# radoslawkrolikowski/financial-market-data-analysis

Hardware: NVIDIA B200
Metric: sequences/sec (train step) biGRU h=256 seq=128 feat=64 (higher is better)
Workload: dtype bf16x3 (fp32-class: split bf16 operand pairs on tensor cores, fp32 accumulate / state / gradients)

## Files before the change

financial_market_data_analysis_b200/csrc/path_x3.cuh:

```cuda
#pragma once
#include "path_bf16.cuh"
#include "tc_scan_x.cuh"
#include <cstdlib>

static int x3_plan_check(const bigru_plan& p) {
    if ((p.H != 128 && p.H != 256) || p.B % 32 != 0) {
        bigru_set_error("BIGRU_PREC_BF16X3 supports hidden_size 128 or 256 and batch %% 32 == 0 (got H=%d B=%d; the Python mirror pads "
                        "other batch sizes with zero rows); use BIGRU_PREC_FP32 for other shapes", p.H, p.B);
        return BIGRU_ERR_UNSUPPORTED;
    }
    return BIGRU_OK;
}

struct X3Layout {
    size_t Yhi[16], Ylo[16], YB[16], G[16], Xhi[16], Xlo[16];
    size_t Wih_hi[16], Wih_lo[16], WihT_hi[16], WihT_lo[16], Wimg[16], WTimg[16], bfold[16], bhn[16];
    size_t cat, arg, dbg, stash_total;
    size_t gi, dghn_hi, dghn_lo, dYa, dYb, gh0, scratch_total;
};
static X3Layout x3_layout(const bigru_plan& p) {
    X3Layout L{};
    const size_t R = (size_t)p.B * p.T, DH = (size_t)p.D * p.H, H = p.H, D = p.D;
    size_t o = 0;
    for (int l = 0; l < p.L; ++l) {
        const size_t I = p.in_size(l), Ip = (size_t)pad8((int64_t)I);
        L.Yhi[l] = o; o = al(o + R * DH * 2);
        L.Ylo[l] = o; o = al(o + R * DH * 2);
        L.YB[l] = o; o = al(o + R * DH * 4);
        L.G[l] = o; o = al(o + R * D * 4 * H * 4);
        L.Xhi[l] = o; o = al(o + R * Ip * 2);
        L.Xlo[l] = o; o = al(o + R * Ip * 2);
        L.Wih_hi[l] = o; o = al(o + D * 3 * H * Ip * 2);
        L.Wih_lo[l] = o; o = al(o + D * 3 * H * Ip * 2);
        L.WihT_hi[l] = o; o = al(o + D * 3 * H * I * 2);
        L.WihT_lo[l] = o; o = al(o + D * 3 * H * I * 2);
        L.Wimg[l] = o; o = al(o + D * 2 * 3 * H * H * 2);
        L.WTimg[l] = o; o = al(o + D * 2 * 3 * H * H * 2);
        L.bfold[l] = o; o = al(o + D * 3 * H * 4);
        L.bhn[l] = o; o = al(o + D * H * 4);
    }
    L.cat = o; o = al(o + (size_t)p.B * 3 * H * 4);
    L.arg = o; o = al(o + (size_t)p.B * H * 4);
    L.dbg = o; o = al(o + 256);
    L.stash_total = o;
    o = 0;
    const size_t wide = DH > (size_t)p.F ? DH : (size_t)p.F;
    L.gi = o; o = al(o + R * D * 3 * H * 4);
    L.dghn_hi = o; o = al(o + R * D * H * 2);
    L.dghn_lo = o; o = al(o + R * D * H * 2);
    L.dYa = o; o = al(o + R * wide * 4);
    L.dYb = o; o = al(o + R * wide * 4);
    L.gh0 = o; o = al(o + (size_t)p.B * D * 3 * H * 4);
    L.scratch_total = o;
    return L;
}
static void x3_workspace(const bigru_plan& p, size_t* a, size_t* b) {
    const X3Layout L = x3_layout(p);
    *a = L.stash_total; *b = L.scratch_total;
}

__device__ __forceinline__ void x3_split(float x, bf16_t& hi, bf16_t& lo) {
    hi = __float2bfloat16(x);
    lo = __float2bfloat16(x - __bfloat162float(hi));
}

__global__ void x3_dropout_rows_kernel(const bf16_t* __restrict__ Yhi, const bf16_t* __restrict__ Ylo, bf16_t* __restrict__ Xhi,
                                       bf16_t* __restrict__ Xlo, int64_t R, int cols, int B, int T, float pdrop, uint64_t seed, uint32_t stream) {
    const float scale = 1.f / (1.f - pdrop);
    const int64_t total = R * cols;
    for (int64_t i = (int64_t)blockIdx.x * blockDim.x + threadIdx.x; i < total; i += (int64_t)gridDim.x * blockDim.x) {
        const int cidx = i % cols;
        const int64_t r = i / cols;
        const int64_t b = r % B, t = r / B;
        const uint64_t key = ((uint64_t)b * T + t) * cols + cidx;
        const float v = bigru_uniform(seed, stream, key) < pdrop ? 0.f : (__bfloat162float(Yhi[i]) + __bfloat162float(Ylo[i])) * scale;
        bf16_t hi, lo;
        x3_split(v, hi, lo);
        Xhi[i] = hi; Xlo[i] = lo;
    }
}
__global__ void x3_dropout_grad_rows_kernel(float* __restrict__ dYB, int64_t R, int cols, int B, int T, int H, float pdrop,
                                            uint64_t seed, uint32_t stream) {
    const float scale = 1.f / (1.f - pdrop);
    const int64_t total = R * cols;
    const int CS = H / 64, ntl = B / 32;
    for (int64_t i = (int64_t)blockIdx.x * blockDim.x + threadIdx.x; i < total; i += (int64_t)gridDim.x * blockDim.x) {
        const int i8 = i & 7;
        int64_t e = i >> 3;
        const int tid = e % 256; e /= 256;
        const int c = e % CS; e /= CS;
        const int t = e % T; e /= T;
        const int tile = e % ntl;
        const int d = e / ntl;
        const int unit = c * 64 + (tid & 63);
        const int64_t b = tile * 32 + (tid >> 6) * 8 + i8;
        const uint64_t key = ((uint64_t)b * T + t) * cols + (uint64_t)(d * H + unit);
        dYB[i] = bigru_uniform(seed, stream, key) < pdrop ? 0.f : dYB[i] * scale;
    }
}

struct X3PackJob { const float* w_ih; const float* w_hh; const float* b_ih; const float* b_hh;
                   bf16_t *Wih_hi, *Wih_lo, *WihT_hi, *WihT_lo, *Wimg, *WTimg; float* bfold; float* bhn; int I; int d; };
struct X3PackJobs { X3PackJob j[32]; };
__global__ void __launch_bounds__(256) x3_pack_all_kernel(const X3PackJobs jobs, int H, int D) {
    __shared__ float tile[32][33];
    const X3PackJob& J = jobs.j[blockIdx.y];
    const int H3 = 3 * H, I = J.I, d = J.d;
    const int tx = threadIdx.x & 31, ty = threadIdx.x >> 5;
    if (I % 32 == 0) {
        const int tr = H3 / 32, tcn = I / 32;
        for (int tl = blockIdx.x; tl < tr * tcn; tl += gridDim.x) {
            const int r0 = (tl / tcn) * 32, c0 = (tl % tcn) * 32;
#pragma unroll
            for (int i = ty; i < 32; i += 8) {
                const float v = J.w_ih[(int64_t)(r0 + i) * I + c0 + tx];
                tile[i][tx] = v;
                bf16_t hi, lo;
                x3_split(v, hi, lo);
                const int64_t o = ((int64_t)d * H3 + r0 + i) * I + c0 + tx;
                J.Wih_hi[o] = hi; J.Wih_lo[o] = lo;
            }
            __syncthreads();
#pragma unroll
            for (int i = ty; i < 32; i += 8) {
                bf16_t hi, lo;
                x3_split(tile[tx][i], hi, lo);
                const int64_t o = (int64_t)(c0 + i) * D * H3 + (int64_t)d * H3 + r0 + tx;
                J.WihT_hi[o] = hi; J.WihT_lo[o] = lo;
            }
            __syncthreads();
        }
    } else {
        const int Ip = (I + 7) & ~7;
        const int64_t n_ih = (int64_t)H3 * Ip;
        for (int64_t i = (int64_t)blockIdx.x * blockDim.x + threadIdx.x; i < n_ih; i += (int64_t)gridDim.x * blockDim.x) {
            const int k = i % Ip, q = i / Ip;
            bf16_t hi, lo;
            x3_split(k < I ? J.w_ih[(int64_t)q * I + k] : 0.f, hi, lo);
            const int64_t o1 = ((int64_t)d * H3 + q) * Ip + k, o2 = (int64_t)k * D * H3 + (int64_t)d * H3 + q;
            J.Wih_hi[o1] = hi; J.Wih_lo[o1] = lo;
            if (k < I) { J.WihT_hi[o2] = hi; J.WihT_lo[o2] = lo; }
        }
    }
    {
        const int CS = H / 64, NKH = H / 128, NRB = 2 * NKH;
        const int64_t per_cta = (int64_t)128 * 3 * H;
        const int64_t total = (int64_t)CS * per_cta;
        bf16_t* fimg = J.Wimg + (int64_t)d * total;
        bf16_t* bimg = J.WTimg + (int64_t)d * total;
        for (int64_t i = (int64_t)blockIdx.x * blockDim.x + threadIdx.x; i < total; i += (int64_t)gridDim.x * blockDim.x) {
            const int c = (int)(i / per_cta);
            const int64_t r = i % per_cta;
            {
                const int row = (int)(r / (3 * H)), col = (int)(r % (3 * H));
                const int g = col / H, k = col % H, part = row >> 6, jj = row & 63;
                bf16_t hi, lo;
                x3_split(J.w_hh[((int64_t)g * H + 64 * c + jj) * H + k], hi, lo);
                fimg[i] = part ? lo : hi;
            }
            {
                const int lane_i = (int)(r / (NRB * 192)), col = (int)(r % (NRB * 192));
                const int rb = col / 192, kq = col % 192, g = kq / 64, jj = kq % 64;
                const int part = rb / NKH, kh = rb % NKH;
                bf16_t hi, lo;
                x3_split(J.w_hh[((int64_t)g * H + 64 * c + jj) * H + 128 * kh + lane_i], hi, lo);
                bimg[i] = part ? lo : hi;
            }
        }
    }
    for (int64_t q = (int64_t)blockIdx.x * blockDim.x + threadIdx.x; q < H3; q += (int64_t)gridDim.x * blockDim.x) {
        J.bfold[d * H3 + q] = J.b_ih[q] + (q < 2 * H ? J.b_hh[q] : 0.f);
        if (q >= 2 * H) J.bhn[d * H + q - 2 * H] = J.b_hh[q];
    }
}

static int forward_x3(const bigru_plan& p, const float* params, const float* x, const float* h0, float drop,
                      int spatial, int training, uint64_t seed, void* stash_v, void* scratch_v, float* logits,
                      float* hn, cudaStream_t st, WindowSrc win = WindowSrc{nullptr, nullptr, nullptr, 0}) {
    const X3Layout L = x3_layout(p);
    uint8_t* S = (uint8_t*)stash_v;
    uint8_t* W = (uint8_t*)scratch_v;
    const int B = p.B, T = p.T, H = p.H, D = p.D, F = p.F;
    const int64_t R = (int64_t)B * T;
    const bool do_drop = training && drop > 0.f;
    unsigned int* dbg = (unsigned int*)(S + L.dbg);
    CUDA_TRY(cudaMemsetAsync(dbg, 0, 64, st));
    {
        X3PackJobs jobs{};
        int nj = 0;
        for (int l = 0; l < p.L; ++l)
            for (int d = 0; d < D; ++d) {
                X3PackJob& J = jobs.j[nj++];
                J.w_ih = params + p.off_wih(l, d); J.w_hh = params + p.off_whh(l, d);
                J.b_ih = params + p.off_bih(l, d); J.b_hh = params + p.off_bhh(l, d);
                J.Wih_hi = (bf16_t*)(S + L.Wih_hi[l]); J.Wih_lo = (bf16_t*)(S + L.Wih_lo[l]);
                J.WihT_hi = (bf16_t*)(S + L.WihT_hi[l]); J.WihT_lo = (bf16_t*)(S + L.WihT_lo[l]);
                J.Wimg = (bf16_t*)(S + L.Wimg[l]); J.WTimg = (bf16_t*)(S + L.WTimg[l]);
                J.bfold = (float*)(S + L.bfold[l]); J.bhn = (float*)(S + L.bhn[l]); J.I = (int)p.in_size(l); J.d = d;
            }
        KLAUNCH(KC_PACK, 0.0, 0.0, st, x3_pack_all_kernel<<<dim3(148, nj), 256, 0, st>>>(jobs, H, D));
    }
    const bool direct = windows_direct(p, win.src != nullptr, do_drop);
    if (direct)
        KLAUNCH(KC_PACK, 0.0, 8.0 * (B + T - 1) * F, st, chunk_prep_kernel<<<148, 256, 0, st>>>(win, (bf16_t*)(S + L.Xhi[0]), (bf16_t*)(S + L.Xlo[0]),
                                                                                                 (int64_t)B + T - 1, F));
    else if (F % 8 == 0)
        KLAUNCH(KC_PACK, 0.0, 8.0 * R * F, st, cast_x_kernel<<<148 * 8, 256, 0, st>>>(x, win, (bf16_t*)(S + L.Xhi[0]), (bf16_t*)(S + L.Xlo[0]), B, T, F,
                                                                                       do_drop ? drop : 0.f, spatial, seed));
    else
        KLAUNCH(KC_PACK, 0.0, 8.0 * R * F, st, cast_x_pad_kernel<<<148 * 8, 256, 0, st>>>(x, win, (bf16_t*)(S + L.Xhi[0]), (bf16_t*)(S + L.Xlo[0]), B, T, F,
                                                                                           pad8(F), do_drop ? drop : 0.f, spatial, seed));
    for (int l = 0; l < p.L; ++l) {
        const int I = (int)p.in_size(l);
        const bf16_t* Xhi = (const bf16_t*)(S + L.Xhi[l]);
        const bf16_t* Xlo = (const bf16_t*)(S + L.Xlo[l]);
        if (l > 0) {
            if (do_drop) {
                KLAUNCH(KC_MISC, 0.0, 0.0, st, x3_dropout_rows_kernel<<<148 * 8, 256, 0, st>>>(
                                                   (const bf16_t*)(S + L.Yhi[l - 1]), (const bf16_t*)(S + L.Ylo[l - 1]), (bf16_t*)(S + L.Xhi[l]),
                                                   (bf16_t*)(S + L.Xlo[l]), R, I, B, T, drop, seed, (uint32_t)l));
            } else {
                Xhi = (const bf16_t*)(S + L.Yhi[l - 1]); Xlo = (const bf16_t*)(S + L.Ylo[l - 1]);
            }
        }
        {
            tcg::Params g{};
            const int Ip = pad8(I);
            g.M = D * 3 * H; g.N = (int)R; g.K = Ip; g.batch = 1; g.splitk = 1; g.mode = tcg::OUT_SCAN_F32;
            g.blk = tcg::ScanBlk{T, B, H, 3, 64, 32}; g.m_fast = 1;
            g.C = W + L.gi; g.ldc = R; g.bias = (const float*)(S + L.bfold[l]); g.bias_per_row = 1; g.dbg = dbg;
            const bool wnd = direct && l == 0;
            g.b_win = wnd ? B : 0;
            TRY(tc_gemm(S + L.Wih_hi[l], D * 3 * H, Ip, Xhi, wnd ? (int64_t)B + T - 1 : R, Ip, g, st, KC_TC_GEMM, S + L.Wih_lo[l], Xlo));
        }
        if (h0) {
            GemmArgs r = gemm_args(h0 + (int64_t)l * D * B * H, params + p.off_whh(l, 0), (float*)(W + L.gh0), B, 3 * H, H, H, 1, H, 1, 3 * H);
            r.batch = D; r.zA = (int64_t)B * H; r.zB = p.ld_block(l); r.zC = (int64_t)B * 3 * H;
            TRY(sgemm_launch(r, st));
        }
        tcx::FwdParams f{};
        f.B = B; f.T = T; f.H = H; f.D = D;
        f.Wimg = (const bf16_t*)(S + L.Wimg[l]); f.giX = (const float*)(W + L.gi); f.b_hn = (const float*)(S + L.bhn[l]);
        f.h0 = h0 ? h0 + (int64_t)l * D * B * H : nullptr;
        f.gh0 = h0 ? (const float*)(W + L.gh0) : nullptr;
        f.GX = (float*)(S + L.G[l]); f.YBX = (float*)(S + L.YB[l]);
        f.hn_out = hn ? hn + (int64_t)l * D * B * H : nullptr;
        f.Yhi = (bf16_t*)(S + L.Yhi[l]); f.Ylo = (bf16_t*)(S + L.Ylo[l]); f.dbg = dbg;
        {
            ProfScope ps(KC_TC_SCAN_FWD, 2.0 * 3 * H * H * (double)R * D, 0.0, st);
            CUDA_TRY(tcx::launch_fwd(f, st));
        }
    }
    {
        const int G = 256 / (H / 8);
        const size_t hsm = sizeof(float) * ((size_t)3 * G * H + (size_t)p.C * 8);
        KLAUNCH(KC_HEAD, 0.0, 4.0 * R * D * H, st, head_fwd_kernel<<<B, 256, hsm, st>>>(
                    (const bf16_t*)(S + L.Yhi[p.L - 1]), (const bf16_t*)(S + L.Ylo[p.L - 1]), params + p.off_linw(), params + p.off_linb(),
                    (float*)(S + L.cat), (int*)(S + L.arg), logits, B, T, H, D, p.C));
    }
    return BIGRU_OK;
}

static int backward_x3(const bigru_plan& p, const float* params, const float* x, const float* h0, float drop,
                       int spatial, int training, uint64_t seed, const void* stash_v, void* scratch_v,
                       const float* dlogits, float* grads, float* dx, float* dh0, cudaStream_t st, int l_from = -1, int l_to = 0) {
    if (l_from < 0) l_from = p.L - 1;
    const bool from_top = l_from == p.L - 1;
    const X3Layout L = x3_layout(p);
    const uint8_t* S = (const uint8_t*)stash_v;
    uint8_t* W = (uint8_t*)scratch_v;
    const int B = p.B, T = p.T, H = p.H, D = p.D, C = p.C;
    const int64_t R = (int64_t)B * T;
    const bool do_drop = training && drop > 0.f;
    unsigned int* dbg = (unsigned int*)(const_cast<uint8_t*>(S) + L.dbg);
    if (from_top) CUDA_TRY(cudaMemsetAsync(grads, 0, sizeof(float) * p.nparams, st));
    const float* cat = (const float*)(S + L.cat);
    if (from_top) {
        const int bchunk = 16;
        KLAUNCH(KC_HEAD, 0.0, 0.0, st, head_bwd_w_kernel<<<dim3(nblk2(3 * H, 128), C, (B + bchunk - 1) / bchunk), 128, 0, st>>>(
                    dlogits, cat, grads + p.off_linw(), grads + p.off_linb(), B, 3 * H, C, bchunk));
    }
    float* dY = (float*)(W + L.dYa);
    float* dYnext = (float*)(W + L.dYb);
    if ((p.L - 1 - l_from) & 1) { float* t_ = dY; dY = dYnext; dYnext = t_; }
    bf16_t* dgi_hi = (bf16_t*)(W + L.gi);
    bf16_t* dgi_lo = dgi_hi + (size_t)R * D * 3 * H;
    bf16_t* dghn_hi = (bf16_t*)(W + L.dghn_hi);
    bf16_t* dghn_lo = (bf16_t*)(W + L.dghn_lo);
    for (int l = l_from; l >= l_to; --l) {
        const int I = (int)p.in_size(l);
        tcx::BwdParams b{};
        b.B = B; b.T = T; b.H = H; b.D = D;
        b.WTimg = (const bf16_t*)(S + L.WTimg[l]); b.GX = (const float*)(S + L.G[l]); b.YBX = (const float*)(S + L.YB[l]);
        b.dYBX = dY;
        b.h0 = h0 ? h0 + (int64_t)l * D * B * H : nullptr;
        b.dh0 = dh0 ? dh0 + (int64_t)l * D * B * H : nullptr;
        if (l == p.L - 1) { b.dlogits = dlogits; b.lin_w = params + p.off_linw(); b.arg = (const int*)(S + L.arg); b.C = C; }
        b.dgi_hi = dgi_hi; b.dgi_lo = dgi_lo; b.dghn_hi = dghn_hi; b.dghn_lo = dghn_lo;
        b.db_ih = grads + p.off_bih(l, 0); b.db_hh = grads + p.off_bhh(l, 0); b.dir_stride = p.ld_block(l); b.dbg = dbg;
        {
            ProfScope ps(KC_TC_SCAN_BWD, 2.0 * 3 * H * H * (double)R * D, 0.0, st);
            CUDA_TRY(tcx::launch_bwd(b, st));
        }
        const bool dropped = do_drop && (l == 0 || p.L > 1);
        const bool own_x = l == 0 || dropped;
        const bf16_t* Xin_hi = own_x ? (const bf16_t*)(S + L.Xhi[l]) : (const bf16_t*)(S + L.Yhi[l - 1]);
        const bf16_t* Xin_lo = own_x ? (const bf16_t*)(S + L.Xlo[l]) : (const bf16_t*)(S + L.Ylo[l - 1]);
        {
            tcg::Params g{};
            g.M = 3 * H; g.N = I; g.K = (int)R; g.batch = D; g.mode = tcg::OUT_ATOMIC_F32; g.a_mn = 1; g.b_mn = 1;
            const int tiles = ((3 * H + 127) / 128) * ((I + 127) / 128) * D;
            g.splitk = (int)std::max<int64_t>(1, std::min<int64_t>((R + 63) / 64, (148 * 2 + tiles / 2) / tiles));
            g.C = grads + p.off_wih(l, 0); g.ldc = I; g.zC = p.ld_block(l);
            for (int d = 0; d < D; ++d) { g.a_row_off[d] = d * 3 * H; g.b_row_off[d] = 0; g.b_k_off[d] = 0; }
            g.dbg = dbg;
            g.b_win = (l == 0 && windows_direct(p, x == nullptr, do_drop)) ? B : 0;
            g.b_win_rows = B + T - 1;
            TRY(tc_gemm(dgi_hi, (int64_t)D * 3 * H, (int64_t)D * 3 * H, Xin_hi, I, pad8(I), g, st, KC_TC_GEMM_DWIH, dgi_lo, Xin_lo));
        }
        for (int part = 0; part < 2; ++part) {
            tcg::Params g{};
            g.M = part == 0 ? 2 * H : H; g.N = H; g.K = (int)R; g.batch = D; g.mode = tcg::OUT_ATOMIC_F32; g.a_mn = 1; g.b_mn = 1;
            const int tiles = ((g.M + 127) / 128) * ((H + 127) / 128) * D;
            g.splitk = (int)std::max<int64_t>(1, std::min<int64_t>((R + 63) / 64, (148 * 2 + tiles / 2) / tiles));
            g.C = grads + p.off_whh(l, 0) + (part == 0 ? 0 : (int64_t)2 * H * H); g.ldc = H; g.zC = p.ld_block(l);
            for (int d = 0; d < D; ++d) {
                g.a_row_off[d] = part == 0 ? d * 3 * H : d * H;
                g.b_row_off[d] = d * H; g.b_k_off[d] = d == 0 ? -B : B;
            }
            g.dbg = dbg;
            if (part == 0) TRY(tc_gemm(dgi_hi, (int64_t)D * 3 * H, (int64_t)D * 3 * H, S + L.Yhi[l], (int64_t)D * H, (int64_t)D * H, g, st, KC_TC_GEMM_DWHH, dgi_lo, S + L.Ylo[l]));
            else TRY(tc_gemm(dghn_hi, (int64_t)D * H, (int64_t)D * H, S + L.Yhi[l], (int64_t)D * H, (int64_t)D * H, g, st, KC_TC_GEMM_DWHH, dghn_lo, S + L.Ylo[l]));
        }
        if (h0)
            KLAUNCH(KC_MISC, 0.0, 0.0, st, dwhh_h0_kernel<<<dim3((3 * H + 127) / 128, H / DWHH_H0_COLS, D), 128, 0, st>>>(
                        dgi_hi, dgi_lo, dghn_hi, dghn_lo, h0 + (int64_t)l * D * B * H, grads + p.off_whh(l, 0), p.ld_block(l), B, T, H, D));
        const bool need_dx = l > 0 || dx != nullptr;
        if (need_dx) {
            tcg::Params g{};
            g.M = I; g.N = (int)R; g.K = D * 3 * H; g.batch = 1; g.splitk = 1;
            g.mode = l > 0 ? tcg::OUT_SCAN_F32 : tcg::OUT_F32;
            g.blk = tcg::ScanBlk{T, B, H, 1, 64, 32}; g.m_fast = 1;
            g.C = dYnext; g.ldc = R; g.dbg = dbg;
            TRY(tc_gemm(S + L.WihT_hi[l], I, (int64_t)D * 3 * H, dgi_hi, R, (int64_t)D * 3 * H, g, st, KC_TC_GEMM_DX, S + L.WihT_lo[l], dgi_lo));
            if (l > 0 && dropped)
                KLAUNCH(KC_MISC, 0.0, 0.0, st, x3_dropout_grad_rows_kernel<<<148 * 8, 256, 0, st>>>(dYnext, R, I, B, T, H, drop, seed, (uint32_t)l));
            if (l == 0) {
                dim3 grid((I + 31) / 32, (B + 31) / 32, T);
                KLAUNCH(KC_MISC, 0.0, 0.0, st, dx_to_batch_major_kernel<<<grid, dim3(32, 8), 0, st>>>(dYnext, dx, B, T, I,
                                                                                               do_drop ? drop : 0.f, spatial, seed));
            }
        }
        float* tmp = dY; dY = dYnext; dYnext = tmp;
    }
    return BIGRU_OK;
}
```

financial_market_data_analysis_b200/csrc/tc_gemm.cuh:

```cuda
#pragma once
#include "tc_common.cuh"
#include <cstring>

namespace tcg {

constexpr int BM = 128, BN = 128, BK = 64, MAX_STAGES = 4;
constexpr int A_BYTES = BM * BK * 2, B_BYTES = BN * BK * 2;
static inline int smem_bytes_for(int stages, int stage_out = 65536) {
    const int ring = stages * (A_BYTES + B_BYTES);
    return (ring < stage_out ? stage_out : ring) + 1024  + 256 ;
}
constexpr int THREADS = 192;

enum { OUT_F32 = 0, OUT_BF16 = 1, OUT_ATOMIC_F32 = 2, OUT_SCAN_BF16 = 3, OUT_SCAN_F32 = 4 };

struct ScanBlk { int T, B, H, G; int U, NB; };

struct Params {
    int M, N, K;
    int batch, splitk;
    int mode;
    void* C; int64_t ldc;
    int64_t zC;
    int a_row_off[4], b_row_off[4], b_k_off[4];
// ... 84 lines not shown
                if (++s == STAGES) { s = 0; ph ^= 1; }
            }
        }
    } else if (warp == 1) {
        if (tc::elect_one()) {
            const uint32_t idesc = tc::umma_idesc_bf16(BM, BN, (uint32_t)p.a_mn, (uint32_t)p.b_mn);
            const int nit = nkb * p.nsplit;
            int s = 0;
            uint32_t ph = 0;
            for (int i = 0; i < nit; ++i, s = (s + 1 == STAGES ? 0 : s + 1), ph ^= (s == 0 ? 1u : 0u)) {
                if (!tc::mbar_wait(&full[s], ph, p.dbg, 0x200 + s)) break;
                tc::tcgen05_fence_after();
                const uint32_t aa = tc::smem_u32(sA + s * A_BYTES), ab = tc::smem_u32(sB + s * B_BYTES);
                const uint64_t da = p.a_mn ? tc::umma_desc_mn_sw128(aa, A_BYTES / 2) : tc::umma_desc_k_sw128(aa);
                const uint64_t db = p.b_mn ? tc::umma_desc_mn_sw128(ab, B_BYTES / 2) : tc::umma_desc_k_sw128(ab);
                const uint64_t sa = p.a_mn ? 128 : 2, sb = p.b_mn ? 128 : 2;
#pragma unroll
                for (int kk = 0; kk < BK / 16; ++kk)
                    tc::umma_bf16(tmem, da + sa * kk, db + sb * kk, idesc, (i | kk) ? 1u : 0u);
                tc::umma_commit(&empty[s]);
            }
            tc::umma_commit(accum);
        }
    } else {
        const int q = warp & 3;
        const int m = m0 + q * 32 + lane;
        bool ok = tc::mbar_wait(accum, 0, p.dbg, 0x300);
        tc::tcgen05_fence_after();
        const float* bias = p.bias ? p.bias + z * p.zBias : nullptr;
        const float brow = (bias && p.bias_per_row && m < p.M) ? bias[m] : 0.f;
        if (ok && p.mode >= OUT_SCAN_BF16 && p.tma_store) {
            const int ml = q * 32 + lane;
            const bool bf = p.mode == OUT_SCAN_BF16;
            const int run_bytes = bf ? 2048 : 4096;
#pragma unroll 1
            for (int c = 0; c < BN / 32; ++c) {
                uint32_t v[32];
                if (nkb > 0) { tc::tmem_ld32(tmem + ((uint32_t)(q * 32) << 16) + c * 32, v); tc::tmem_ld_wait(); }
                else {
#pragma unroll
                    for (int i = 0; i < 32; ++i) v[i] = 0u;
                }
                const int nb = n0 + c * 32;
#pragma unroll
                for (int i8 = 0; i8 < 32; i8 += 8) {
                    float f[8];
#pragma unroll
                    for (int j = 0; j < 8; ++j)
                        f[j] = __uint_as_float(v[i8 + j]) + (bias ? (p.bias_per_row ? brow : ((nb + i8 + j < p.N) ? bias[nb + i8 + j] : 0.f)) : 0.f);
                    uint8_t* dst = smem + (size_t)(c * 4 + (i8 >> 3)) * run_bytes;
                    if (bf) {
                        uint32_t w[4];
#pragma unroll
                        for (int j = 0; j < 4; ++j) {
                            __nv_bfloat162 h2 = __floats2bfloat162_rn(f[2 * j], f[2 * j + 1]);
                            w[j] = *reinterpret_cast<uint32_t*>(&h2);
                        }
                        tc::sts_u4(tc::smem_u32(dst) + ml * 16, make_uint4(w[0], w[1], w[2], w[3]));
                    } else {
                        tc::sts_f4(tc::smem_u32(dst) + ml * 32, make_float4(f[0], f[1], f[2], f[3]));
                        tc::sts_f4(tc::smem_u32(dst) + ml * 32 + 16, make_float4(f[4], f[5], f[6], f[7]));
                    }
                }
            }
            tc::fence_proxy_async_smem();
            asm volatile("bar.sync 1, 128;" ::: "memory");
            if (warp == 2 && tc::elect_one()) {
                const int H = p.blk.H, G = p.blk.G, Bb = p.blk.B, Tt = p.blk.T, U = p.blk.U;
                const int sh = p.blk.NB == 32 ? 5 : 4;
                const int CSs = H / U, ntl = Bb >> sh, nh = BM / U;
                const size_t es = bf ? 2 : 4;
                size_t row_part[2]; size_t gate_part[2];
                for (int hh = 0; hh < nh; ++hh) {
                    const int mr = m0 + hh * U;
                    row_part[hh] = (size_t)(mr / (G * H)) * ntl;
                    gate_part[hh] = (size_t)((mr % H) / U) * G + (size_t)((mr / H) % G);
                }
                int t_ = n0 / Bb, b = n0 % Bb;
                for (int r = 0; r < BN / 8; ++r) {
                    if (n0 + r * 8 >= p.N) break;
                    const int tile_ = b >> sh, cbg = (b & ((1 << sh) - 1)) >> 3;
                    for (int hh = 0; hh < nh; ++hh) {
                        const size_t e = ((((row_part[hh] + tile_) * Tt + t_) * CSs * G + gate_part[hh]) * 256 + (size_t)cbg * U) * 8;
                        tc::bulk_s2g(reinterpret_cast<uint8_t*>(p.C) + e * es, smem + (size_t)r * run_bytes + (size_t)hh * U * 8 * es,
                                     (uint32_t)(U * 8 * es));
                    }
                    b += 8;
                    if (b >= Bb) { b -= Bb; ++t_; }
                }
                tc::tma_store_commit();
                tc::tma_store_wait_read();
            }
        } else if (ok && p.tma_store) {
            const int ml = q * 32 + lane;
            const uint32_t sw = (uint32_t)(ml & 7);
            const bool is_bf16 = p.mode == OUT_BF16;
#pragma unroll 1
            for (int c = 0; c < BN / 32; ++c) {
                uint32_t v[32];
                if (nkb > 0) {
                    tc::tmem_ld32(tmem + ((uint32_t)(q * 32) << 16) + c * 32, v);
                    tc::tmem_ld_wait();
                } else {
#pragma unroll
                    for (int i = 0; i < 32; ++i) v[i] = 0u;
                }
                const int nb = n0 + c * 32;
                if (bias && ks == 0) {
#pragma unroll
                    for (int i = 0; i < 32; ++i) {
                        const float bb = p.bias_per_row ? brow : ((nb + i < p.N) ? bias[nb + i] : 0.f);
                        v[i] = __float_as_uint(__uint_as_float(v[i]) + bb);
                    }
                }
                if (is_bf16) {
                    uint8_t* box = smem + (size_t)(c >> 1) * 16384 + (size_t)ml * 128;
#pragma unroll
                    for (int k4 = 0; k4 < 4; ++k4) {
                        uint32_t w[4];
#pragma unroll
                        for (int j = 0; j < 4; ++j) {
                            __nv_bfloat162 h2 = __floats2bfloat162_rn(__uint_as_float(v[k4 * 8 + 2 * j]), __uint_as_float(v[k4 * 8 + 2 * j + 1]));
                            w[j] = *reinterpret_cast<uint32_t*>(&h2);
                        }
                        const uint32_t chunk = ((uint32_t)((c & 1) * 4 + k4)) ^ sw;
                        tc::sts_u4(tc::smem_u32(box) + chunk * 16, make_uint4(w[0], w[1], w[2], w[3]));
                    }
                } else {
                    uint8_t* box = smem + (size_t)c * 16384 + (size_t)ml * 128;
#pragma unroll
                    for (int k4 = 0; k4 < 8; ++k4) {
                        const uint32_t chunk = ((uint32_t)k4) ^ sw;
                        tc::sts_u4(tc::smem_u32(box) + chunk * 16, make_uint4(v[k4 * 4], v[k4 * 4 + 1], v[k4 * 4 + 2], v[k4 * 4 + 3]));
                    }
                }
            }
            tc::fence_proxy_async_smem();
            asm volatile("bar.sync 1, 128;" ::: "memory");
            if (warp == 2 && tc::elect_one()) {
                const int nboxes = is_bf16 ? BN / 64 : BN / 32;
                const int bw = is_bf16 ? 64 : 32;
                for (int b = 0; b < nboxes; ++b) {
                    if (n0 + b * bw >= p.N) break;
                    if (p.mode == OUT_ATOMIC_F32) {
                        if (z == 0) tc::tma_reduce_add_2d(&tmC0, smem + (size_t)b * 16384, n0 + b * bw, m0);
                        else tc::tma_reduce_add_2d(&tmC1, smem + (size_t)b * 16384, n0 + b * bw, m0);
                    } else {
                        if (z == 0) tc::tma_store_2d(&tmC0, smem + (size_t)b * 16384, n0 + b * bw, m0);
                        else tc::tma_store_2d(&tmC1, smem + (size_t)b * 16384, n0 + b * bw, m0);
                    }
                }
                tc::tma_store_commit();
                tc::tma_store_wait_read();
            }
        } else if (ok) {
#pragma unroll 1
            for (int c = 0; c < BN / 32; ++c) {
                uint32_t v[32];
                if (nkb > 0) {
                    tc::tmem_ld32(tmem + ((uint32_t)(q * 32) << 16) + c * 32, v);
                    tc::tmem_ld_wait();
                } else {
#pragma unroll
                    for (int i = 0; i < 32; ++i) v[i] = 0u;
                }
                const int nb = n0 + c * 32;
                if (m < p.M && nb < p.N && p.mode >= OUT_SCAN_BF16) {
                    const int H = p.blk.H, G = p.blk.G, Bb = p.blk.B, Tt = p.blk.T, U = p.blk.U, NBt = p.blk.NB;
                    const int dd = m / (G * H), gg = (m / H) % G, unit = m % H;
                    const int CSs = H / U, cc = unit / U, ju = unit % U;
                    const int ntl = Bb / NBt;
#pragma unroll
                    for (int i8 = 0; i8 < 32; i8 += 8) {
                        const int n = nb + i8;
                        if (n >= p.N) break;
                        const int t = n / Bb, b = n % Bb;
                        const int tile = b / NBt;
                        const int tid = ju + U * ((b % NBt) >> 3);
                        const size_t e = ((((((size_t)dd * ntl + tile) * Tt + t) * CSs + cc) * G + gg) * 256 + tid) * 8;
                        float f[8];
#pragma unroll
                        for (int j = 0; j < 8; ++j) f[j] = __uint_as_float(v[i8 + j]) + (bias ? (p.bias_per_row ? brow : bias[n + j]) : 0.f);
                        if (p.mode == OUT_SCAN_BF16) {
                            uint32_t w[4];
#pragma unroll
                            for (int j = 0; j < 4; ++j) {
                                __nv_bfloat162 h2 = __floats2bfloat162_rn(f[2 * j], f[2 * j + 1]);
                                w[j] = *reinterpret_cast<uint32_t*>(&h2);
                            }
                            *reinterpret_cast<uint4*>(reinterpret_cast<__nv_bfloat16*>(p.C) + e) = make_uint4(w[0], w[1], w[2], w[3]);
                        } else {
                            float4* o = reinterpret_cast<float4*>(reinterpret_cast<float*>(p.C) + e);
                            o[0] = make_float4(f[0], f[1], f[2], f[3]);
                            o[1] = make_float4(f[4], f[5], f[6], f[7]);
                        }
                    }
                } else if (m < p.M && nb < p.N) {
                    if (p.mode == OUT_BF16) {
                        __nv_bfloat16* crow = reinterpret_cast<__nv_bfloat16*>(p.C) + z * p.zC + (int64_t)m * p.ldc + nb;
                        if (nb + 32 <= p.N && (p.ldc % 8 == 0)) {
#pragma unroll
                            for (int i = 0; i < 32; i += 8) {
                                uint32_t w[4];
#pragma unroll
                                for (int j = 0; j < 4; ++j) {
                                    float a = __uint_as_float(v[i + 2 * j]), b = __uint_as_float(v[i + 2 * j + 1]);
                                    if (bias) {
                                        if (p.bias_per_row) { a += brow; b += brow; }
                                        else { a += bias[nb + i + 2 * j]; b += bias[nb + i + 2 * j + 1]; }
                                    }
                                    __nv_bfloat162 h2 = __floats2bfloat162_rn(a, b);
                                    w[j] = *reinterpret_cast<uint32_t*>(&h2);
                                }
                                *reinterpret_cast<uint4*>(crow + i) = make_uint4(w[0], w[1], w[2], w[3]);
                            }
                        } else {
                            for (int i = 0; i < 32 && nb + i < p.N; ++i) {
                                float a = __uint_as_float(v[i]);
                                if (bias) a += p.bias_per_row ? brow : bias[nb + i];
                                crow[i] = __float2bfloat16(a);
                            }
                        }
                    } else {
                        float* crow = reinterpret_cast<float*>(p.C) + z * p.zC + (int64_t)m * p.ldc + nb;
                        for (int i = 0; i < 32 && nb + i < p.N; ++i) {
                            float a = __uint_as_float(v[i]);
                            if (bias && ks == 0) a += p.bias_per_row ? brow : bias[nb + i];
                            if (p.mode == OUT_ATOMIC_F32) atomicAdd(crow + i, a);
                            else crow[i] = a;
                        }
                    }
                }
            }
        }
    }
    tc::tcgen05_fence_before();
    __syncthreads();
    if (warp == 1) tc::tmem_dealloc(tmem, BN);
}

static inline int make_operand_map(CUtensorMap* m, const void* base, uint64_t rows, uint64_t K, uint64_t ld) {
    const uint64_t dims[2] = {K, rows};
    const uint64_t strides[1] = {ld * 2};
    const uint32_t box[2] = {(uint32_t)BK, 128u};
    return make_tmap_bf16(m, base, 2, dims, strides, box);
}

static inline int make_output_map(CUtensorMap* m, void* base, int mode, uint64_t M, uint64_t N, uint64_t ldc) {
    const bool bf = mode == OUT_BF16;
    const uint64_t dims[2] = {N, M};
    const uint64_t strides[1] = {ldc * (bf ? 2u : 4u)};
    const uint32_t box[2] = {bf ? 64u : 32u, 128u};
    return make_tmap_typed(m, bf ? CU_TENSOR_MAP_DATA_TYPE_BFLOAT16 : CU_TENSOR_MAP_DATA_TYPE_FLOAT32, base, 2, dims, strides, box);
}

static inline int make_operand_map_mn(CUtensorMap* m, const void* base, uint64_t Krows, uint64_t MN, uint64_t ld) {
    const uint64_t dims[2] = {MN, Krows};
    const uint64_t strides[1] = {ld * 2};
    const uint32_t box[2] = {64u, (uint32_t)BK};
    return make_tmap_bf16(m, base, 2, dims, strides, box);
}

static inline cudaError_t launch(const CUtensorMap& tmA, const CUtensorMap& tmB, const Params& p_in, cudaStream_t st,
                                 const CUtensorMap* tmAlo = nullptr, const CUtensorMap* tmBlo = nullptr) {
    {
        static bool attr_set[64] = {};
        int dev = 0;
        cudaGetDevice(&dev);
        if (dev < 0 || dev >= 64 || !attr_set[dev]) {
            cudaError_t e = cudaFuncSetAttribute(gemm_kernel, cudaFuncAttributeMaxDynamicSharedMemorySize, smem_bytes_for(MAX_STAGES));
            if (e != cudaSuccess) return e;
            if (dev >= 0 && dev < 64) attr_set[dev] = true;
        }
    }
    Params p = p_in;
    if (p.nsplit != 3 || !tmAlo || !tmBlo) p.nsplit = 1;
    if (p.blk.U == 0) { p.blk.U = 128; p.blk.NB = 16; }
    {
        const int kblocks = (((p.K + BK - 1) / BK + p.splitk - 1) / p.splitk) * p.nsplit;
        p.stages = kblocks <= 2 ? kblocks : (kblocks <= 12 ? 2 : 3);
        if (p.stages < 1) p.stages = 1;
    }
    CUtensorMap tmC[2];
    memset(tmC, 0, sizeof(tmC));
    const size_t es = p.mode == OUT_BF16 ? 2 : 4;
    const bool scan_mode = p.mode >= OUT_SCAN_BF16;
    bool tma_ok = !scan_mode && p.batch <= 2 && ((p.ldc * es) % 16 == 0) && ((p.zC * es) % 16 == 0) && ((uintptr_t)p.C % 16 == 0);
    if (tma_ok) {
        for (int z = 0; z < p.batch; ++z)
            if (make_output_map(&tmC[z], (uint8_t*)p.C + (size_t)z * p.zC * es, p.mode, (uint64_t)p.M, (uint64_t)p.N, (uint64_t)p.ldc) != 0) tma_ok = false;
        if (p.batch == 1) tmC[1] = tmC[0];
    }
    p.tma_store = tma_ok ? 1 : 0;
    if (scan_mode && p.M % BM == 0 && p.blk.H % p.blk.U == 0 && p.blk.B % p.blk.NB == 0 && ((uintptr_t)p.C % 16 == 0)) p.tma_store = 1;
    dim3 grid((p.N + BN - 1) / BN, (p.M + BM - 1) / BM, p.batch * p.splitk);
    if (p.m_fast) { const unsigned t = grid.x; grid.x = grid.y; grid.y = t; }
    const int stage_out = p.tma_store ? ((p.mode == OUT_BF16 || p.mode == OUT_SCAN_BF16) ? 32768 : 65536) : 0;
    gemm_kernel<<<grid, THREADS, smem_bytes_for(p.stages, stage_out), st>>>(tmA, tmB, p.nsplit == 3 ? *tmAlo : tmA, p.nsplit == 3 ? *tmBlo : tmB,
                                                                            tmC[0], tmC[1], p);
    return cudaGetLastError();
}

}
```

Baseline: 164,300.

## Add persistent stream-K bf16x3 GEMM kernel for backward weight and dx GEMMs

Adds a dedicated persistent bf16x3 GEMM kernel with one CTA per SM. Its scheduler uses stream-K for atomic-accumulate outputs and grid-stride over tiles otherwise, with a double-buffered TMEM accumulator so the epilogue overlaps the next tile's MMAs. The two dW_hh GEMMs (r/z gates from dgi, n gate from dghn) are merged into one launch through a second A operand selected by row offset. The dW_ih and dx GEMMs are routed through the new kernel. This is meant to cut split-K launch and wave-quantization overhead and to save a launch, at the cost of a new kernel path with fixed stage counts and 1 CTA/SM occupancy.

After: 154,100, median of 6. -6.2%, worse.

```diff
diff --git a/financial_market_data_analysis_b200/csrc/path_x3.cuh b/financial_market_data_analysis_b200/csrc/path_x3.cuh
--- a/financial_market_data_analysis_b200/csrc/path_x3.cuh
+++ b/financial_market_data_analysis_b200/csrc/path_x3.cuh
@@ -174,6 +174,28 @@
     }
 }
 
+struct X3Operand { const void* hi; const void* lo; int64_t rows, ld; };
+static int x3_operand_map(CUtensorMap* m, const void* base, int mn, int64_t rows, int64_t kext, int64_t ld) {
+    const int e = mn ? tcg::make_operand_map_mn(m, base, (uint64_t)kext, (uint64_t)rows, (uint64_t)ld)
+                     : tcg::make_operand_map(m, base, (uint64_t)rows, (uint64_t)kext, (uint64_t)ld);
+    if (e) bigru_set_error("cuTensorMapEncodeTiled failed (rows %lld K %lld ld %lld)", (long long)rows, (long long)kext, (long long)ld);
+    return e;
+}
+static int tc_gemm_x3(const X3Operand& A, const X3Operand& Bo, tcg::X3Params& p, cudaStream_t st, int kclass,
+                      const X3Operand& A2 = X3Operand{nullptr, nullptr, 0, 0}) {
+    CUtensorMap tA, tAl, tB, tBl, tA2, tA2l;
+    const int64_t bk = p.b_mn && p.b_win ? p.b_win_rows : p.K;
+    if (x3_operand_map(&tA, A.hi, p.a_mn, A.rows, p.K, A.ld) || x3_operand_map(&tAl, A.lo, p.a_mn, A.rows, p.K, A.ld) ||
+        x3_operand_map(&tB, Bo.hi, p.b_mn, Bo.rows, bk, Bo.ld) || x3_operand_map(&tBl, Bo.lo, p.b_mn, Bo.rows, bk, Bo.ld))
+        return BIGRU_ERR_CUDA;
+    const bool a2 = A2.hi != nullptr;
+    if (a2 && (x3_operand_map(&tA2, A2.hi, p.a_mn, A2.rows, p.K, A2.ld) || x3_operand_map(&tA2l, A2.lo, p.a_mn, A2.rows, p.K, A2.ld)))
+        return BIGRU_ERR_CUDA;
+    ProfScope ps(kclass, 2.0 * p.M * p.N * (double)p.K * p.batch, 0.0, st);
+    CUDA_TRY(tcg::launch_x3(tA, tAl, tB, tBl, a2 ? &tA2 : nullptr, a2 ? &tA2l : nullptr, p, st));
+    return BIGRU_OK;
+}
+
 static int forward_x3(const bigru_plan& p, const float* params, const float* x, const float* h0, float drop,
                       int spatial, int training, uint64_t seed, void* stash_v, void* scratch_v, float* logits,
                       float* hn, cudaStream_t st, WindowSrc win = WindowSrc{nullptr, nullptr, nullptr, 0}) {
@@ -307,42 +329,41 @@
         const bf16_t* Xin_hi = own_x ? (const bf16_t*)(S + L.Xhi[l]) : (const bf16_t*)(S + L.Yhi[l - 1]);
         const bf16_t* Xin_lo = own_x ? (const bf16_t*)(S + L.Xlo[l]) : (const bf16_t*)(S + L.Ylo[l - 1]);
         {
-            tcg::Params g{};
+            tcg::X3Params g{};
             g.M = 3 * H; g.N = I; g.K = (int)R; g.batch = D; g.mode = tcg::OUT_ATOMIC_F32; g.a_mn = 1; g.b_mn = 1;
-            const int tiles = ((3 * H + 127) / 128) * ((I + 127) / 128) * D;
-            g.splitk = (int)std::max<int64_t>(1, std::min<int64_t>((R + 63) / 64, (148 * 2 + tiles / 2) / tiles));
             g.C = grads + p.off_wih(l, 0); g.ldc = I; g.zC = p.ld_block(l);
             for (int d = 0; d < D; ++d) { g.a_row_off[d] = d * 3 * H; g.b_row_off[d] = 0; g.b_k_off[d] = 0; }
             g.dbg = dbg;
             g.b_win = (l == 0 && windows_direct(p, x == nullptr, do_drop)) ? B : 0;
             g.b_win_rows = B + T - 1;
-            TRY(tc_gemm(dgi_hi, (int64_t)D * 3 * H, (int64_t)D * 3 * H, Xin_hi, I, pad8(I), g, st, KC_TC_GEMM_DWIH, dgi_lo, Xin_lo));
-        }
-        for (int part = 0; part < 2; ++part) {
-            tcg::Params g{};
-            g.M = part == 0 ? 2 * H : H; g.N = H; g.K = (int)R; g.batch = D; g.mode = tcg::OUT_ATOMIC_F32; g.a_mn = 1; g.b_mn = 1;
-            const int tiles = ((g.M + 127) / 128) * ((H + 127) / 128) * D;
-            g.splitk = (int)std::max<int64_t>(1, std::min<int64_t>((R + 63) / 64, (148 * 2 + tiles / 2) / tiles));
-            g.C = grads + p.off_whh(l, 0) + (part == 0 ? 0 : (int64_t)2 * H * H); g.ldc = H; g.zC = p.ld_block(l);
+            TRY(tc_gemm_x3(X3Operand{dgi_hi, dgi_lo, (int64_t)D * 3 * H, (int64_t)D * 3 * H}, X3Operand{Xin_hi, Xin_lo, I, pad8(I)},
+                           g, st, KC_TC_GEMM_DWIH));
+        }
+        {
+            tcg::X3Params g{};
+            g.M = 3 * H; g.N = H; g.K = (int)R; g.batch = D; g.mode = tcg::OUT_ATOMIC_F32; g.a_mn = 1; g.b_mn = 1;
+            g.C = grads + p.off_whh(l, 0); g.ldc = H; g.zC = p.ld_block(l);
+            g.a2_m = 2 * H;
             for (int d = 0; d < D; ++d) {
-                g.a_row_off[d] = part == 0 ? d * 3 * H : d * H;
+                g.a_row_off[d] = d * 3 * H; g.a2_row_off[d] = d * H;
                 g.b_row_off[d] = d * H; g.b_k_off[d] = d == 0 ? -B : B;
             }
             g.dbg = dbg;
-            if (part == 0) TRY(tc_gemm(dgi_hi, (int64_t)D * 3 * H, (int64_t)D * 3 * H, S + L.Yhi[l], (int64_t)D * H, (int64_t)D * H, g, st, KC_TC_GEMM_DWHH, dgi_lo, S + L.Ylo[l]));
-            else TRY(tc_gemm(dghn_hi, (int64_t)D * H, (int64_t)D * H, S + L.Yhi[l], (int64_t)D * H, (int64_t)D * H, g, st, KC_TC_GEMM_DWHH, dghn_lo, S + L.Ylo[l]));
+            TRY(tc_gemm_x3(X3Operand{dgi_hi, dgi_lo, (int64_t)D * 3 * H, (int64_t)D * 3 * H}, X3Operand{S + L.Yhi[l], S + L.Ylo[l], (int64_t)D * H, (int64_t)D * H},
+                           g, st, KC_TC_GEMM_DWHH, X3Operand{dghn_hi, dghn_lo, (int64_t)D * H, (int64_t)D * H}));
         }
         if (h0)
             KLAUNCH(KC_MISC, 0.0, 0.0, st, dwhh_h0_kernel<<<dim3((3 * H + 127) / 128, H / DWHH_H0_COLS, D), 128, 0, st>>>(
                         dgi_hi, dgi_lo, dghn_hi, dghn_lo, h0 + (int64_t)l * D * B * H, grads + p.off_whh(l, 0), p.ld_block(l), B, T, H, D));
         const bool need_dx = l > 0 || dx != nullptr;
         if (need_dx) {
-            tcg::Params g{};
+            tcg::X3Params g{};
             g.M = I; g.N = (int)R; g.K = D * 3 * H; g.batch = 1; g.splitk = 1;
             g.mode = l > 0 ? tcg::OUT_SCAN_F32 : tcg::OUT_F32;
             g.blk = tcg::ScanBlk{T, B, H, 1, 64, 32}; g.m_fast = 1;
             g.C = dYnext; g.ldc = R; g.dbg = dbg;
-            TRY(tc_gemm(S + L.WihT_hi[l], I, (int64_t)D * 3 * H, dgi_hi, R, (int64_t)D * 3 * H, g, st, KC_TC_GEMM_DX, S + L.WihT_lo[l], dgi_lo));
+            TRY(tc_gemm_x3(X3Operand{S + L.WihT_hi[l], S + L.WihT_lo[l], I, (int64_t)D * 3 * H}, X3Operand{dgi_hi, dgi_lo, R, (int64_t)D * 3 * H},
+                           g, st, KC_TC_GEMM_DX));
             if (l > 0 && dropped)
                 KLAUNCH(KC_MISC, 0.0, 0.0, st, x3_dropout_grad_rows_kernel<<<148 * 8, 256, 0, st>>>(dYnext, R, I, B, T, H, drop, seed, (uint32_t)l));
             if (l == 0) {
diff --git a/financial_market_data_analysis_b200/csrc/tc_gemm.cuh b/financial_market_data_analysis_b200/csrc/tc_gemm.cuh
--- a/financial_market_data_analysis_b200/csrc/tc_gemm.cuh
+++ b/financial_market_data_analysis_b200/csrc/tc_gemm.cuh
@@ -410,3 +410,5 @@
 }
 
 }
+
+#include "tc_gemm_x3.cuh"
diff --git a/financial_market_data_analysis_b200/csrc/tc_gemm_x3.cuh b/financial_market_data_analysis_b200/csrc/tc_gemm_x3.cuh
--- /dev/null
+++ b/financial_market_data_analysis_b200/csrc/tc_gemm_x3.cuh
@@ -0,0 +1,295 @@
+#pragma once
+#include "tc_gemm.cuh"
+
+namespace tcg {
+
+struct X3Params : Params {
+    int a2_m;
+    int a2_row_off[4];
+};
+
+constexpr int X3_TILE = BM * BK * 2;
+constexpr int X3_STAGE_BYTES = 4 * X3_TILE;
+constexpr int X3_STG_BYTES = 16384;
+constexpr int X3_DATA = 3 * X3_STAGE_BYTES + 2 * X3_STG_BYTES;
+constexpr int X3_SMEM = X3_DATA + 1024  + 256 ;
+static_assert(X3_SMEM <= 227 * 1024 && X3_DATA == 2 * X3_STAGE_BYTES + 6 * X3_STG_BYTES, "x3 GEMM shared memory");
+constexpr int X3_SHORT_KB = 8;
+constexpr int X3_SK_PIECE = 128;
+
+struct X3Sched {
+    int tiles_m, tiles_n, kbt, slices;
+    int64_t ntile;
+    int64_t pos, end, stride;
+    bool sk;
+    __device__ __forceinline__ X3Sched(const X3Params& p) {
+        tiles_m = (p.M + BM - 1) / BM; tiles_n = (p.N + BN - 1) / BN; kbt = (p.K + BK - 1) / BK;
+        ntile = (int64_t)tiles_m * tiles_n * p.batch;
+        sk = p.mode == OUT_ATOMIC_F32;
+        slices = 1;
+        if (sk) {
+            slices = (int)min((int64_t)kbt, (gridDim.x + ntile - 1) / ntile);
+            const int64_t total = ntile * kbt;
+            pos = total * blockIdx.x / gridDim.x; end = total * (blockIdx.x + 1) / gridDim.x; stride = 0;
+        } else {
+            pos = blockIdx.x; end = ntile; stride = gridDim.x;
+        }
+    }
+    __device__ __forceinline__ bool next(const X3Params& p, int& z, int& m0, int& n0, int& kb0, int& nkb) {
+        int64_t tile;
+        if (sk) {
+            if (pos >= end) return false;
+            const int64_t q = pos / ntile;
+            const int sl = (int)min((int64_t)slices - 1, ((q + 1) * slices - 1) / kbt);
+            const int ks0 = (int)((int64_t)sl * kbt / slices), ks1 = (int)((int64_t)(sl + 1) * kbt / slices);
+            const int64_t r = pos - ntile * ks0;
+            tile = r / (ks1 - ks0);
+            const int kl = (int)(r % (ks1 - ks0));
+            kb0 = ks0 + kl;
+            nkb = (int)min((int64_t)min(ks1 - ks0 - kl, X3_SK_PIECE), end - pos);
+            pos += nkb;
+        } else {
+            if (pos >= end) return false;
+            tile = pos; kb0 = 0; nkb = kbt;
+            pos += stride;
+        }
+        int mt, nt;
+        if (p.m_fast) { mt = (int)(tile % tiles_m); tile /= tiles_m; nt = (int)(tile % tiles_n); tile /= tiles_n; }
+        else { nt = (int)(tile % tiles_n); tile /= tiles_n; mt = (int)(tile % tiles_m); tile /= tiles_m; }
+        z = (int)tile; m0 = mt * BM; n0 = nt * BN;
+        return true;
+    }
+};
+
+__device__ __forceinline__ void x3_load(uint8_t* dst, const CUtensorMap* m, uint64_t* bar, int mn, int row, int k) {
+    if (mn) { tc::tma_load_2d(dst, m, bar, row, k); tc::tma_load_2d(dst + X3_TILE / 2, m, bar, row + 64, k); }
+    else tc::tma_load_2d(dst, m, bar, k, row);
+}
+
+__global__ void __launch_bounds__(THREADS, 1)
+gemm_x3_kernel(const __grid_constant__ CUtensorMap tmA, const __grid_constant__ CUtensorMap tmAlo,
+               const __grid_constant__ CUtensorMap tmB, const __grid_constant__ CUtensorMap tmBlo,
+               const __grid_constant__ CUtensorMap tmA2, const __grid_constant__ CUtensorMap tmA2lo,
+               const __grid_constant__ CUtensorMap tmC0, const __grid_constant__ CUtensorMap tmC1, const X3Params p) {
+    extern __shared__ uint8_t smem_raw[];
+    uint8_t* smem = reinterpret_cast<uint8_t*>((reinterpret_cast<uintptr_t>(smem_raw) + 1023) & ~uintptr_t(1023));
+    const int STAGES = p.stages, NSTG = STAGES == 2 ? 6 : 2;
+    uint8_t* stg = smem + STAGES * X3_STAGE_BYTES;
+    uint64_t* bars = reinterpret_cast<uint64_t*>(smem + X3_DATA);
+    uint64_t* full = bars;
+    uint64_t* empty = bars + 3;
+    uint64_t* acc_full = bars + 6;
+    uint64_t* acc_empty = bars + 8;
+    uint32_t* tmem_slot = reinterpret_cast<uint32_t*>(bars + 10);
+
+    const int warp = threadIdx.x >> 5, lane = threadIdx.x & 31;
+    if (threadIdx.x == 0) {
+        for (int s = 0; s < STAGES; ++s) { tc::mbar_init(&full[s], 1); tc::mbar_init(&empty[s], 1); }
+        for (int a = 0; a < 2; ++a) { tc::mbar_init(&acc_full[a], 1); tc::mbar_init(&acc_empty[a], 4); }
+        tc::fence_mbar_init();
+    }
+    if (warp == 1) tc::tmem_alloc(tmem_slot, 2 * BN);
+    tc::tcgen05_fence_before();
+    __syncthreads();
+    tc::tcgen05_fence_after();
+    const uint32_t tmem = *tmem_slot;
+    X3Sched sched(p);
+    int z, m0, n0, kb0, nkb;
+
+    if (warp == 0) {
+        if (tc::elect_one()) {
+            tc::tma_prefetch_desc(&tmA); tc::tma_prefetch_desc(&tmAlo);
+            tc::tma_prefetch_desc(&tmB); tc::tma_prefetch_desc(&tmBlo);
+            if (p.a2_m > 0) { tc::tma_prefetch_desc(&tmA2); tc::tma_prefetch_desc(&tmA2lo); }
+            int s = 0;
+            uint32_t ph = 0;
+            bool ok = true;
+            while (ok && sched.next(p, z, m0, n0, kb0, nkb)) {
+                const bool a2 = p.a2_m > 0 && m0 >= p.a2_m;
+                const int ar = a2 ? p.a2_row_off[z] + m0 - p.a2_m : p.a_row_off[z] + m0;
+                for (int i = 0; i < nkb; ++i) {
+                    if (!tc::mbar_wait(&empty[s], ph ^ 1, p.dbg, 0x500 + s)) { ok = false; break; }
+                    tc::mbar_arrive_expect_tx(&full[s], X3_STAGE_BYTES);
+                    const int k = (kb0 + i) * BK;
+                    int br = p.b_row_off[z] + n0, kb = k + p.b_k_off[z];
+                    if (p.b_win) { if (p.b_mn) kb = kb / p.b_win + kb % p.b_win; else br = p.b_row_off[z] + n0 / p.b_win + n0 % p.b_win; }
+                    uint8_t* d = smem + s * X3_STAGE_BYTES;
+                    if (a2) { x3_load(d, &tmA2, &full[s], p.a_mn, ar, k); x3_load(d + X3_TILE, &tmA2lo, &full[s], p.a_mn, ar, k); }
+                    else { x3_load(d, &tmA, &full[s], p.a_mn, ar, k); x3_load(d + X3_TILE, &tmAlo, &full[s], p.a_mn, ar, k); }
+                    x3_load(d + 2 * X3_TILE, &tmB, &full[s], p.b_mn, br, kb);
+                    x3_load(d + 3 * X3_TILE, &tmBlo, &full[s], p.b_mn, br, kb);
+                    if (++s == STAGES) { s = 0; ph ^= 1; }
+                }
+            }
+        }
+    } else if (warp == 1) {
+        if (tc::elect_one()) {
+            const uint32_t idesc = tc::umma_idesc_bf16(BM, BN, (uint32_t)p.a_mn, (uint32_t)p.b_mn);
+            const uint64_t sa = p.a_mn ? 128 : 2, sb = p.b_mn ? 128 : 2;
+            int s = 0, it = 0;
+            uint32_t ph = 0;
+            bool ok = true;
+            while (ok && sched.next(p, z, m0, n0, kb0, nkb)) {
+                const int a = it & 1;
+                if (!tc::mbar_wait(&acc_empty[a], ((it >> 1) & 1) ^ 1, p.dbg, 0x580 + a)) break;
+                tc::tcgen05_fence_after();
+                const uint32_t tacc = tmem + (uint32_t)(a * BN);
+                for (int i = 0; i < nkb; ++i) {
+                    if (!tc::mbar_wait(&full[s], ph, p.dbg, 0x600 + s)) { ok = false; break; }
+                    tc::tcgen05_fence_after();
+                    const uint32_t base = tc::smem_u32(smem + s * X3_STAGE_BYTES);
+                    const uint64_t dah = p.a_mn ? tc::umma_desc_mn_sw128(base, X3_TILE / 2) : tc::umma_desc_k_sw128(base);
+                    const uint64_t dal = p.a_mn ? tc::umma_desc_mn_sw128(base + X3_TILE, X3_TILE / 2) : tc::umma_desc_k_sw128(base + X3_TILE);
+                    const uint64_t dbh = p.b_mn ? tc::umma_desc_mn_sw128(base + 2 * X3_TILE, X3_TILE / 2) : tc::umma_desc_k_sw128(base + 2 * X3_TILE);
+                    const uint64_t dbl = p.b_mn ? tc::umma_desc_mn_sw128(base + 3 * X3_TILE, X3_TILE / 2) : tc::umma_desc_k_sw128(base + 3 * X3_TILE);
+#pragma unroll
+                    for (int kk = 0; kk < BK / 16; ++kk) tc::umma_bf16(tacc, dah + sa * kk, dbh + sb * kk, idesc, (i | kk) ? 1u : 0u);
+#pragma unroll
+                    for (int kk = 0; kk < BK / 16; ++kk) tc::umma_bf16(tacc, dah + sa * kk, dbl + sb * kk, idesc, 1u);
+#pragma unroll
+                    for (int kk = 0; kk < BK / 16; ++kk) tc::umma_bf16(tacc, dal + sa * kk, dbh + sb * kk, idesc, 1u);
+                    tc::umma_commit(&empty[s]);
+                    if (++s == STAGES) { s = 0; ph ^= 1; }
+                }
+                tc::umma_commit(&acc_full[a]);
+                ++it;
+            }
+        }
+    } else {
+        const int q = warp & 3, ml = q * 32 + lane;
+        const bool issuer = warp == 2 && lane == 0;
+        const bool scan = p.mode == OUT_SCAN_F32;
+        int it = 0, buf_i = 0;
+        while (sched.next(p, z, m0, n0, kb0, nkb)) {
+            const int a = it & 1;
+            if (!tc::mbar_wait(&acc_full[a], (it >> 1) & 1, p.dbg, 0x700 + a)) break;
+            tc::tcgen05_fence_after();
+            const uint32_t tacc = tmem + (uint32_t)(a * BN) + ((uint32_t)(q * 32) << 16);
+            const int m = m0 + ml;
+            const float brow = (p.bias && kb0 == 0 && m < p.M) ? p.bias[z * p.zBias + m] : 0.f;
+#pragma unroll 1
+            for (int c = 0; c < BN / 32; ++c) {
+                uint32_t v[32];
+                tc::tmem_ld32(tacc + c * 32, v);
+                tc::tmem_ld_wait();
+                if (c == BN / 32 - 1) {
+                    tc::tcgen05_fence_before();
+                    __syncwarp();
+                    if (lane == 0) tc::mbar_arrive(&acc_empty[a]);
+                }
+                const int nb = n0 + c * 32;
+                if (nb >= p.N) continue;
+                if (scan || brow != 0.f) {
+#pragma unroll
+                    for (int i = 0; i < 32; ++i) v[i] = __float_as_uint(__uint_as_float(v[i]) + brow);
+                }
+                if (!p.tma_store) {
+                    if (m < p.M) {
+                        float* crow = reinterpret_cast<float*>(p.C) + z * p.zC + (int64_t)m * p.ldc + nb;
+                        for (int i = 0; i < 32 && nb + i < p.N; ++i) {
+                            if (p.mode == OUT_ATOMIC_F32) atomicAdd(crow + i, __uint_as_float(v[i]));
+                            else crow[i] = __uint_as_float(v[i]);
+                        }
+                    }
+                    continue;
+                }
+                uint8_t* buf = stg + buf_i * X3_STG_BYTES;
+                if (issuer) {
+                    if (NSTG == 6) asm volatile("cp.async.bulk.wait_group.read 5;" ::: "memory");
+                    else asm volatile("cp.async.bulk.wait_group.read 1;" ::: "memory");
+                }
+                asm volatile("bar.sync 1, 128;" ::: "memory");
+                if (scan) {
+#pragma unroll
+                    for (int r = 0; r < 4; ++r) {
+                        const uint32_t dst = tc::smem_u32(buf + r * 4096) + ml * 32;
+                        tc::sts_f4(dst, make_float4(__uint_as_float(v[8 * r]), __uint_as_float(v[8 * r + 1]), __uint_as_float(v[8 * r + 2]), __uint_as_float(v[8 * r + 3])));
+                        tc::sts_f4(dst + 16, make_float4(__uint_as_float(v[8 * r + 4]), __uint_as_float(v[8 * r + 5]), __uint_as_float(v[8 * r + 6]), __uint_as_float(v[8 * r + 7])));
+                    }
+                } else {
+                    const uint32_t row = tc::smem_u32(buf) + ml * 128, sw = (uint32_t)(ml & 7);
+#pragma unroll
+                    for (int k4 = 0; k4 < 8; ++k4) tc::sts_u4(row + ((k4 ^ sw) << 4), make_uint4(v[k4 * 4], v[k4 * 4 + 1], v[k4 * 4 + 2], v[k4 * 4 + 3]));
+                }
+                tc::fence_proxy_async_smem();
+                asm volatile("bar.sync 1, 128;" ::: "memory");
+                if (issuer) {
+                    if (scan) {
+                        const int H = p.blk.H, G = p.blk.G, Bb = p.blk.B, U = p.blk.U;
+                        const int sh = p.blk.NB == 32 ? 5 : 4;
+                        const int ntl = Bb >> sh, nh = BM / U;
+                        for (int hh = 0; hh < nh; ++hh) {
+                            const int mr = m0 + hh * U;
+                            const size_t row_part = (size_t)(mr / (G * H)) * ntl;
+                            const size_t gate_part = (size_t)((mr % H) / U) * G + (size_t)((mr / H) % G);
+                            int t_ = nb / Bb, b = nb % Bb;
+                            for (int r = 0; r < 4 && nb + r * 8 < p.N; ++r) {
+                                const int tile_ = b >> sh, cbg = (b & ((1 << sh) - 1)) >> 3;
+                                const size_t e = ((((row_part + tile_) * p.blk.T + t_) * (H / U) * G + gate_part) * 256 + (size_t)cbg * U) * 8;
+                                tc::bulk_s2g(reinterpret_cast<float*>(p.C) + e, buf + r * 4096 + hh * U * 32, (uint32_t)(U * 32));
+                                b += 8;
+                                if (b >= Bb) { b -= Bb; ++t_; }
+                            }
+                        }
+                    } else if (p.mode == OUT_ATOMIC_F32) {
+                        if (z == 0) tc::tma_reduce_add_2d(&tmC0, buf, nb, m0);
+                        else tc::tma_reduce_add_2d(&tmC1, buf, nb, m0);
+                    } else {
+                        if (z == 0) tc::tma_store_2d(&tmC0, buf, nb, m0);
+                        else tc::tma_store_2d(&tmC1, buf, nb, m0);
+                    }
+                    tc::tma_store_commit();
+                }
+                if (++buf_i == NSTG) buf_i = 0;
+            }
+            ++it;
+        }
+        if (issuer) tc::tma_store_wait_read();
+    }
+    tc::tcgen05_fence_before();
+    __syncthreads();
+    if (warp == 1) tc::tmem_dealloc(tmem, 2 * BN);
+}
+
+static inline cudaError_t launch_x3(const CUtensorMap& tmA, const CUtensorMap& tmAlo, const CUtensorMap& tmB, const CUtensorMap& tmBlo,
+                                    const CUtensorMap* tmA2, const CUtensorMap* tmA2lo, const X3Params& p_in, cudaStream_t st) {
+    int dev = 0;
+    cudaError_t e = cudaGetDevice(&dev);
+    if (e != cudaSuccess) return e;
+    static bool attr_set[64] = {};
+    static int n_sm[64] = {};
+    if (dev < 0 || dev >= 64) return cudaErrorInvalidDevice;
+    if (!attr_set[dev]) {
+        e = cudaFuncSetAttribute(gemm_x3_kernel, cudaFuncAttributeMaxDynamicSharedMemorySize, X3_SMEM);
+        if (e == cudaSuccess) e = cudaDeviceGetAttribute(&n_sm[dev], cudaDevAttrMultiProcessorCount, dev);
+        if (e != cudaSuccess) return e;
+        attr_set[dev] = true;
+    }
+    X3Params p = p_in;
+    const bool scan = p.mode == OUT_SCAN_F32;
+    if (!(scan || p.mode == OUT_F32 || p.mode == OUT_ATOMIC_F32) || (p.bias && !p.bias_per_row) || p.batch < 1 || p.batch > 2 ||
+        p.K < 1 || (p.a2_m > 0 && (p.a2_m % BM != 0 || !tmA2 || !tmA2lo)))
+        return cudaErrorInvalidValue;
+    if (p.blk.U == 0) { p.blk.U = 128; p.blk.NB = 16; }
+    CUtensorMap tmC[2];
+    memset(tmC, 0, sizeof(tmC));
+    if (scan) {
+        if (p.M % BM != 0 || p.blk.H % p.blk.U != 0 || BM % p.blk.U != 0 || p.blk.B % p.blk.NB != 0 || ((uintptr_t)p.C % 16 != 0))
+            return cudaErrorInvalidValue;
+        p.tma_store = 1;
+    } else {
+        bool ok = (p.ldc * 4) % 16 == 0 && (p.zC * 4) % 16 == 0 && ((uintptr_t)p.C % 16 == 0);
+        for (int z = 0; ok && z < p.batch; ++z)
+            ok = make_output_map(&tmC[z], (uint8_t*)p.C + (size_t)z * p.zC * 4, p.mode, (uint64_t)p.M, (uint64_t)p.N, (uint64_t)p.ldc) == 0;
+        if (p.batch == 1) tmC[1] = tmC[0];
+        p.tma_store = ok ? 1 : 0;
+    }
+    p.stages = (p.K + BK - 1) / BK <= X3_SHORT_KB ? 2 : 3;
+    const int64_t tiles = (int64_t)((p.M + BM - 1) / BM) * ((p.N + BN - 1) / BN) * p.batch;
+    const int64_t work = p.mode == OUT_ATOMIC_F32 ? tiles * ((p.K + BK - 1) / BK) : tiles;
+    const unsigned ctas = (unsigned)(work < n_sm[dev] ? work : n_sm[dev]);
+    gemm_x3_kernel<<<ctas, THREADS, X3_SMEM, st>>>(tmA, tmAlo, tmB, tmBlo, tmA2 ? *tmA2 : tmA, tmA2lo ? *tmA2lo : tmAlo, tmC[0], tmC[1], p);
+    return cudaGetLastError();
+}
+
+}
```
